# mandt-lab/PSLD

Measured on AMD Instinct MI355X. Metric: train images/sec, CIFAR-10 PSLD (6ch 32x32) NCSN++ HSM step, higher is better.
Workload: dtype f32

## Files before the change

psld_amd/csrc/conv_wino.hip:

```cpp
#include <cstdlib>
#include <cstring>
#include <type_traits>

#include "common.h"
#include "psld_hip.h"
#include "tile_shared.h"
#include "limb.h"

namespace {

constexpr int WT = 32;
constexpr int VPLANE = WT * ROWB;
constexpr int VBYTES = 16 * 3 * VPLANE;
constexpr int WINO_THREADS = 512;

struct WinoArgs {
    const float* x1;
    const float* x2;
    int C1, C2;
    int B, H, W;
    const u32x4* ufrag;
    int N, M;
    int chunks;
    float* C;
    int ldc;
    int nseg, rps;
    int cw;
    PsldEpilogue e;
    const float* zero;
    int nmajor;
    int tiles_m;
    int stagger;
    const float *gsc1, *gsh1, *gsc2, *gsh2;
    int gn_act;
    unsigned long long* dbg;
    int lg_tiles_x, lg_tps;
    int ksplit;
    long long slab_stride;
    int lg_ksplit, lg_xblocks;
    int lg_rpi;
    int mul_seg, mul_w2;
    int rb_img;
    float opscale;
};

constexpr int wino_mul16(int d) { return 65536 / d + 1; }
__host__ __device__ constexpr int wino_div16(int x, int mul) { return (x * mul) >> 16; }
constexpr int WINO_GEOS[7][2] = {{4, 4}, {4, 8}, {8, 8}, {16, 8}, {4, 16}, {8, 16}, {4, 32}};
constexpr bool wino_div16_exact() {
    for (const auto& g : WINO_GEOS) {
        const int W2 = g[1] + 2, seg_px = (g[0] + 2) * W2;
        for (int x = 0; x < 256; ++x)
            if (wino_div16(x, wino_mul16(seg_px)) != x / seg_px || wino_div16(x, wino_mul16(W2)) != x / W2) return false;
    }
    return true;
}
static_assert(wino_div16_exact(), "halo decomposition: multiply-shift must equal the division for every pixel below 256");
constexpr bool wino_geo_listed(int rps, int cw) {
    for (const auto& g : WINO_GEOS)
        if (g[0] == rps && g[1] == cw) return true;
    return false;
}
constexpr int wino_lg2(int v) {
    int l = 0;
    while ((1 << l) < v) ++l;
    return (1 << l) == v ? l : -1;
}

__device__ __forceinline__ int raw_off(int hp, int q) {
    return (hp >> 1) * 256 + (((((hp & 1) ^ ((hp >> 1) & 1)) << 3) + q) << 4);
}

template <int NL = 3>
__device__ __forceinline__ void wino_pack_item(const float* __restrict__ w, u32x4* __restrict__ out, long long it, int k_in,
                                               long long sn, long long sk, int flip) {
    const int chunks = k_in / 32;
    long long t = it;
    const int lane = (int)(t & 63); t >>= 6;
    const int chunk = (int)(t % chunks); t /= chunks;
    const int nblk = (int)t;
    const int n = nblk * 16 + (lane & 15);
    const int k0 = chunk * 32 + (lane >> 4) * 8;
    float U[8][16];
#pragma unroll
    for (int j = 0; j < 8; ++j) {
        const float* p = w + n * sn + (k0 + j) * sk;
        float g[3][3];
#pragma unroll
        for (int a = 0; a < 3; ++a)
#pragma unroll
            for (int b = 0; b < 3; ++b) g[a][b] = flip ? p[8 - (a * 3 + b)] : p[a * 3 + b];
        float t4[4][3];
#pragma unroll
        for (int b = 0; b < 3; ++b) {
            t4[0][b] = g[0][b];
            t4[1][b] = 0.5f * ((g[0][b] + g[2][b]) + g[1][b]);
            t4[2][b] = 0.5f * ((g[0][b] + g[2][b]) - g[1][b]);
            t4[3][b] = g[2][b];
        }
#pragma unroll
        for (int a = 0; a < 4; ++a) {
            U[j][a * 4 + 0] = t4[a][0];
            U[j][a * 4 + 1] = 0.5f * ((t4[a][0] + t4[a][2]) + t4[a][1]);
            U[j][a * 4 + 2] = 0.5f * ((t4[a][0] + t4[a][2]) - t4[a][1]);
            U[j][a * 4 + 3] = t4[a][2];
        }
    }
    u32x4* o = out + ((long long)nblk * chunks + chunk) * (16 * NL * 64) + lane;
#pragma unroll
    for (int p = 0; p < 16; ++p) {
        unsigned hi[4], mid[4], lo[4];
#pragma unroll
        for (int j = 0; j < 4; ++j) {
            if constexpr (NL == 3) split3(U[2 * j][p], U[2 * j + 1][p], hi[j], mid[j], lo[j]);
            else if constexpr (NL == 2) split2(U[2 * j][p], U[2 * j + 1][p], hi[j], mid[j]);
            else hi[j] = cvt_pk_f16(U[2 * j][p], U[2 * j + 1][p]);
        }
        o[(p * NL + 0) * 64] = u32x4{hi[0], hi[1], hi[2], hi[3]};
        if constexpr (NL >= 2) o[(p * NL + 1) * 64] = u32x4{mid[0], mid[1], mid[2], mid[3]};
        if constexpr (NL == 3) o[(p * 3 + 2) * 64] = u32x4{lo[0], lo[1], lo[2], lo[3]};
    }
}

template <int NL = 3>
__global__ void wino_pack_kernel(const float* __restrict__ w, u32x4* __restrict__ out, int n_out, int k_in,
                                 long long sn, long long sk, int flip) {
    const long long items = (long long)(n_out / 16) * (k_in / 32) * 64;
    for (long long it = (long long)blockIdx.x * blockDim.x + threadIdx.x; it < items; it += (long long)gridDim.x * blockDim.x)
        wino_pack_item<NL>(w, out, it, k_in, sn, sk, flip);
}

template <int NL = 3>
__global__ void wino_pack_batch_kernel(const long long* __restrict__ tab, int ntab, long long total) {
    for (long long idx = (long long)blockIdx.x * blockDim.x + threadIdx.x; idx < total;
         idx += (long long)gridDim.x * blockDim.x) {
        int lo = 0, hi = ntab - 1;
        while (lo < hi) {
            const int mid = (lo + hi + 1) >> 1;
            if (tab[8 * mid + 7] <= idx) lo = mid; else hi = mid - 1;
        }
        const long long* d = tab + 8 * lo;
        wino_pack_item<NL>(reinterpret_cast<const float*>(d[0]), reinterpret_cast<u32x4*>(d[1]), idx - d[7], (int)d[3], d[5], d[6],
                       (int)d[4]);
    }
}

template <int ABL = 0, bool GNF = false, bool ERAW = false, int LA = 2, bool TAIL = false, int NL = 3, bool SH = false>
__global__ void __launch_bounds__(WINO_THREADS) wino_conv8s_kernel(const WinoArgs a) {
    extern __shared__ __attribute__((aligned(16))) unsigned char smem[];
    constexpr int NI = 4;
    constexpr int RAWB = NI * 64 * 128;
    unsigned char* Vs = smem;
    unsigned char* Rs = smem + VBYTES / 3 * NL;

    const int tid = threadIdx.x;
    const int lane = tid & 63, wave = __builtin_amdgcn_readfirstlane(tid >> 6);
    const int tiles_n = TAIL ? (a.N + 127) >> 7 : a.N >> 7;
    const int nsp = a.ksplit > 1 ? a.ksplit : 1;
    const int tiles_m = a.tiles_m;
    const int per_range = tiles_m * tiles_n;
    const int vb = xcd_remap(blockIdx.x, gridDim.x);
    const int split = nsp > 1 ? vb / per_range : 0;
    const int bid = vb - split * per_range;
    const int kch = a.chunks >> a.lg_ksplit, ch0 = split * kch;
    float* const Cw = a.C + split * a.slab_stride;
    const int tile_n = a.nmajor ? bid / tiles_m : bid % tiles_n;
    const int tile_m = a.nmajor ? bid - tile_n * tiles_m : bid / tiles_n;
    const int n0 = tile_n * 128;
    const bool live = !TAIL || n0 + wave * 16 < a.N;

    const int HW = a.H * a.W;
    const int W2 = a.cw + 2;
    const int lg_tx = a.lg_tiles_x, lg_tps = a.lg_tps;
    const int rpi = HW >= 128 ? HW >> 7 : 1;
    const int tm_img = a.lg_rpi >= 0 ? tile_m >> a.lg_rpi : tile_m / rpi;
    const int reg = tile_m - tm_img * rpi;
    const int img0 = HW >= 128 ? tm_img : tile_m * a.nseg;
    const int oy0 = (reg >> a.lg_xblocks) * a.rps, ox0 = (reg & ((1 << a.lg_xblocks) - 1)) * a.cw;
    const float* zp = a.zero;

    const int c4 = tid & 7;
    int hoff[NI], rdst[NI];
    {
        const int seg_px = (a.rps + 2) * W2;
#pragma unroll
        for (int i = 0; i < NI; ++i) {
            const int px = (tid + WINO_THREADS * i) >> 3;
            const int seg = wino_div16(px, a.mul_seg);
            const int rem = px - seg * seg_px;
            const int hr = wino_div16(rem, a.mul_w2), hx = rem - hr * W2;
            const int img = img0 + seg, iy = oy0 + hr - 1, ix = ox0 + hx - 1;
            const bool ok = seg < a.nseg && img < a.B && iy >= 0 && iy < a.H && ix >= 0 && ix < a.W;
            hoff[i] = ok ? (img * a.H + iy) * a.W + ix : -1;
            rdst[i] = raw_off(px, c4);
        }
    }
    f32x4 hv[NI];
    auto load_raw = [&](int c) {
        const int c0 = c * 32;
        const bool second = c0 >= a.C1;
        const float* src = second ? a.x2 : a.x1;
        const int cs = second ? a.C2 : a.C1;
        const int cc = (second ? c0 - a.C1 : c0) + c4 * 4;
#pragma unroll
        for (int i = 0; i < NI; ++i) hv[i] = ld4(hoff[i] >= 0 ? src + ((long long)hoff[i] * cs + cc) : zp);
    };
    auto store_raw = [&](int buf, int c) {
        if constexpr (GNF) {
            const int c0 = c * 32;
            const bool second = c0 >= a.C1;
            const int cs = second ? a.C2 : a.C1;
            const long long go = (long long)img0 * cs + (second ? c0 - a.C1 : c0) + c4 * 4;
            const f32x4 sc = ld4((second ? a.gsc2 : a.gsc1) + go), sh = ld4((second ? a.gsh2 : a.gsh1) + go);
#pragma unroll
            for (int i = 0; i < NI; ++i) {
                f32x4 o;
#pragma unroll
                for (int e = 0; e < 4; ++e) {
                    const float z = hv[i][e] * sc[e] + sh[e];
                    const float v = a.gn_act ? silu_f(z) : z;
                    o[e] = hoff[i] >= 0 ? v : 0.f;
                }
                *reinterpret_cast<f32x4*>(Rs + buf * RAWB + rdst[i]) = o;
            }
        } else {
#pragma unroll
            for (int i = 0; i < NI; ++i) *reinterpret_cast<f32x4*>(Rs + buf * RAWB + rdst[i]) = hv[i];
        }
    };

    const int vr = wave >> 2;
    const int t_tile = (tid & 255) >> 3, t_q = tid & 7;
    int t_src;
    {
        const int seg = t_tile >> lg_tps, rem = t_tile & ((1 << lg_tps) - 1);
        const int ty = rem >> lg_tx, tx = rem & ((1 << lg_tx) - 1);
        t_src = seg < a.nseg ? (seg * (a.rps + 2) + 2 * ty) * W2 + 2 * tx : 0;
    }
    const int t_dst = t_tile * ROWB + (((t_q >> 1) ^ lds_swz(t_tile)) << 4) + (t_q & 1) * 8;
    int t_ro[3][4];
#pragma unroll
    for (int k = 0; k < 3; ++k)
#pragma unroll
        for (int c = 0; c < 4; ++c) {
            t_ro[k][c] = raw_off(t_src + (vr + k) * W2 + c, t_q);
            asm volatile("" : "+v"(t_ro[k][c]));
        }
    auto transform = [&](auto TH, auto VR, int rbuf) {
        constexpr int th = decltype(TH)::value, v_r = decltype(VR)::value;
        constexpr int ra_ = th == 0 ? (v_r == 0 ? 0 : 1) : (v_r == 0 ? 2 : 1);
        constexpr int rb_ = th == 0 ? 2 : (v_r == 0 ? 1 : 3);
        constexpr bool plus = th == 0 && v_r == 1;
        constexpr int vrow = 2 * th + v_r;
        const unsigned char* Rb = Rs + rbuf * RAWB;
        f32x4 ea[4], eb[4];
#pragma unroll
        for (int c = 0; c < 4; ++c) {
            ea[c] = *reinterpret_cast<const f32x4*>(Rb + t_ro[ra_ - v_r][c]);
            eb[c] = *reinterpret_cast<const f32x4*>(Rb + t_ro[rb_ - v_r][c]);
        }
        f32x4 r[4];
#pragma unroll
        for (int c = 0; c < 4; ++c) r[c] = plus ? ea[c] + eb[c] : ea[c] - eb[c];
#pragma unroll
        for (int j = 0; j < 4; ++j) {
            const f32x4 v = j == 0 ? r[0] - r[2] : j == 1 ? r[1] + r[2] : j == 2 ? r[2] - r[1] : r[1] - r[3];
            unsigned h0, m0_, l0, h1, m1, l1;
            if constexpr (NL == 3) {
                split3(v[0], v[1], h0, m0_, l0);
                split3(v[2], v[3], h1, m1, l1);
            } else if constexpr (NL == 2) {
                split2(v[0], v[1], h0, m0_);
                split2(v[2], v[3], h1, m1);
            } else if constexpr (SH) {
                h0 = cvt_pk_f16(v[0] * a.opscale, v[1] * a.opscale);
                h1 = cvt_pk_f16(v[2] * a.opscale, v[3] * a.opscale);
            } else {
                h0 = cvt_pk_f16(v[0], v[1]);
                h1 = cvt_pk_f16(v[2], v[3]);
            }
            unsigned char* q = Vs + (vrow * 4 + j) * NL * VPLANE + t_dst;
            *reinterpret_cast<u32x2*>(q) = u32x2{h0, h1};
            if constexpr (NL >= 2) *reinterpret_cast<u32x2*>(q + VPLANE) = u32x2{m0_, m1};
            if constexpr (NL == 3) *reinterpret_cast<u32x2*>(q + 2 * VPLANE) = u32x2{l0, l1};
        }
    };

    const int r16 = lane & 15, kq = lane >> 4;
    int aoff[2];
#pragma unroll
    for (int tb = 0; tb < 2; ++tb) {
        const int row = tb * 16 + r16;
        aoff[tb] = row * ROWB + ((kq ^ lds_swz(row)) << 4);
    }
    const u32x4* ub = a.ufrag + ((long long)(tile_n * 8 + ((ABL & 128) ? (wave & 3) : wave)) * a.chunks + ch0) * (16 * NL * 64);
    u32x4 bq[4][NL];
    auto load_b = [&](int sigma, u32x4 (&dst)[NL]) {
        const u32x4* p = ub + (long long)sigma * (NL * 64);
#pragma unroll
        for (int l = 0; l < NL; ++l) dst[l] = p[l * 64 + lane];
    };
    f32x4v acc[16][2];
#pragma unroll
    for (int p = 0; p < 16; ++p)
#pragma unroll
        for (int tb = 0; tb < 2; ++tb) acc[p][tb] = f32x4v{0.f, 0.f, 0.f, 0.f};
    u32x4 fa[NL == 1 ? 2 : NL][2];
    auto read_a = [&](int p, int l) {
#pragma unroll
        for (int tb = 0; tb < 2; ++tb) fa[l][tb] = *reinterpret_cast<const u32x4*>(Vs + (p * NL + l) * VPLANE + aoff[tb]);
    };
    auto mm = [&](int p, int la, int lb) {
#pragma unroll
        for (int tb = 0; tb < 2; ++tb) {
            if constexpr (NL == 1)
                acc[p][tb] = __builtin_amdgcn_mfma_f32_16x16x32_f16(
                    __builtin_bit_cast(f16x8, bq[p & 3][lb]), __builtin_bit_cast(f16x8, fa[la][tb]), acc[p][tb], 0, 0, 0);
            else
                acc[p][tb] = __builtin_amdgcn_mfma_f32_16x16x32_bf16(
                    __builtin_bit_cast(bf16x8, bq[p & 3][lb]), __builtin_bit_cast(bf16x8, fa[la][tb]), acc[p][tb], 0, 0, 0);
        }
    };
    auto mfma_half = [&](auto HH, auto LAST, int c) {
        constexpr int h = decltype(HH)::value;
        constexpr bool last = decltype(LAST)::value;
        if constexpr ((ABL & 256) != 0) __builtin_amdgcn_s_setprio(2);
        if constexpr (NL == 1) {
            auto read_a1 = [&](int p) {
#pragma unroll
                for (int tb = 0; tb < 2; ++tb) fa[p & 1][tb] = *reinterpret_cast<const u32x4*>(Vs + p * VPLANE + aoff[tb]);
            };
            read_a1(8 * h);
#pragma unroll
            for (int i = 0; i < 8; ++i) {
                const int p = 8 * h + i;
                if (!(last && p + LA >= 16)) load_b(c * 16 + p + LA, bq[(p + LA) & 3]);
                if (i < 7) read_a1(p + 1);
                __builtin_amdgcn_sched_barrier(0);
                mm(p, p & 1, 0);
                __builtin_amdgcn_sched_barrier(0);
            }
            return;
        }
        if constexpr (NL == 3) read_a(8 * h, 2);
        if constexpr (NL >= 2) read_a(8 * h, 1);
        read_a(8 * h, 0);
#pragma unroll
        for (int i = 0; i < 8; ++i) {
            const int p = 8 * h + i;
            if (!(ABL & 2) && !(last && p + LA >= 16)) load_b(c * 16 + p + LA, bq[(p + LA) & 3]);
            __builtin_amdgcn_sched_barrier(0);
            if constexpr (NL == 3) {
                mm(p, 2, 0);
                __builtin_amdgcn_sched_barrier(0);
                if (i < 7) read_a(p + 1, 2);
                __builtin_amdgcn_sched_barrier(0);
                mm(p, 1, 1);
            }
            if constexpr (NL >= 2) {
                mm(p, 1, 0);
                __builtin_amdgcn_sched_barrier(0);
                if (i < 7) read_a(p + 1, 1);
                __builtin_amdgcn_sched_barrier(0);
            }
            if constexpr (NL == 3) mm(p, 0, 2);
            if constexpr (NL >= 2) mm(p, 0, 1);
            mm(p, 0, 0);
            __builtin_amdgcn_sched_barrier(0);
            if (i < 7) read_a(p + 1, 0);
        }
        if constexpr ((ABL & 256) != 0) __builtin_amdgcn_s_setprio(0);
    };
    using I0 = std::integral_constant<int, 0>;
    using I1 = std::integral_constant<int, 1>;
    if constexpr ((ABL & 4) == 0 && (ABL & 256) == 0) { if (vr != 0) __builtin_amdgcn_s_setprio(1); }

    load_raw(ch0);
    if (live) {
        load_b(0, bq[0]);
        load_b(1, bq[1]);
        if (LA > 2) load_b(2, bq[2]);
    }
    store_raw(0, ch0);
    if constexpr (ERAW) load_raw(ch0 + min(1, kch - 1));
    __syncthreads();
    if (vr == 0) transform(I0{}, I0{}, 0); else transform(I0{}, I1{}, 0);
    __syncthreads();

    auto stamp = [&](int c, int idx) {
        if constexpr ((ABL & 64) != 0) {
            if (c == 3 && a.dbg) {
                __builtin_amdgcn_sched_barrier(0);
                const unsigned long long t = __builtin_amdgcn_s_memtime();
                if (lane == 0) a.dbg[((long long)blockIdx.x * 8 + wave) * 8 + idx] = t;
                __builtin_amdgcn_sched_barrier(0);
            }
        }
    };
    using No = std::false_type;
    using Yes = std::true_type;

    for (int c = 0; c < kch - 1; ++c) {
        stamp(c, 0);
        if constexpr (!ERAW) load_raw(ch0 + c + 1);
        if (vr == 0 && !(ABL & 1)) transform(I1{}, I0{}, c & 1);
        __builtin_amdgcn_sched_barrier(0);
        if (vr == 0) stamp(c, 1);
        if (live) mfma_half(I0{}, No{}, c);
        __builtin_amdgcn_sched_barrier(0);
        if (vr != 0) stamp(c, 1);
        if (vr != 0 && !(ABL & 1)) transform(I1{}, I1{}, c & 1);
        stamp(c, 2);
        store_raw((c + 1) & 1, ch0 + c + 1);
        stamp(c, 3);
        __syncthreads();
        stamp(c, 4);
        if (vr == 0 && !(ABL & 1)) transform(I0{}, I0{}, (c + 1) & 1);
        __builtin_amdgcn_sched_barrier(0);
        if (vr == 0) stamp(c, 5);
        if (live) mfma_half(I1{}, No{}, c);
        __builtin_amdgcn_sched_barrier(0);
        if (vr != 0) stamp(c, 5);
        if constexpr (ERAW) load_raw(ch0 + min(c + 2, kch - 1));
        if (vr != 0 && !(ABL & 1)) transform(I0{}, I1{}, (c + 1) & 1);
        stamp(c, 6);
        __syncthreads();
        stamp(c, 7);
    }
    {
        int c = kch - 1;
        asm volatile("" : "+s"(c));
        stamp(c, 0);
        if (vr == 0 && !(ABL & 1)) transform(I1{}, I0{}, c & 1);
        __builtin_amdgcn_sched_barrier(0);
        if (vr == 0) stamp(c, 1);
        if (live) mfma_half(I0{}, No{}, c);
        __builtin_amdgcn_sched_barrier(0);
        if (vr != 0) stamp(c, 1);
        if (vr != 0 && !(ABL & 1)) transform(I1{}, I1{}, c & 1);
        stamp(c, 2);
        stamp(c, 3);
        __syncthreads();
        stamp(c, 4);
        __builtin_amdgcn_sched_barrier(0);
        stamp(c, 5);
        if (live) mfma_half(I1{}, Yes{}, c);
        __builtin_amdgcn_sched_barrier(0);
        stamp(c, 6);
        stamp(c, 7);
    }

    if (!live) return;
    const PsldEpilogue& e = a.e;
    const int cn = n0 + wave * 16 + 4 * kq;
    const int org = (img0 * a.H + oy0) * a.W + ox0;
    const f32x4v zero4 = {0.f, 0.f, 0.f, 0.f};
    const bool rb_div = e.rowbias && !a.rb_img;
    char* const c_b = reinterpret_cast<char*>(Cw + (long long)org * a.ldc);
    const char* const res_b = reinterpret_cast<const char*>(e.res ? e.res + (long long)org * e.ldres : zp);
    f32x4v epi_bias, epi_tbv[2], epi_rv[2][4], epi_cv[2][4];
    int epi_rel[2];
    bool epi_ok[2];
    auto epi_rows = [&](auto TB) {
        constexpr int tb = decltype(TB)::value;
#pragma unroll
        for (int j = 0; j < 4; ++j) {
            const int px = epi_rel[tb] + (j >> 1) * a.W + (j & 1);
            epi_rv[tb][j] = e.res ? *reinterpret_cast<const f32x4v*>(res_b + (unsigned)((px * e.ldres + cn) * 4)) : zero4;
            epi_cv[tb][j] = e.accumulate ? *reinterpret_cast<const f32x4v*>(c_b + (unsigned)((px * a.ldc + cn) * 4)) : zero4;
        }
    };
    auto epi_request = [&]() {
        epi_bias = e.bias ? *reinterpret_cast<const f32x4v*>(e.bias + cn) : zero4;
#pragma unroll
        for (int tb = 0; tb < 2; ++tb) {
            const int tile = tb * 16 + r16;
            const int seg = tile >> lg_tps, rem = tile & ((1 << lg_tps) - 1);
            const int ty = rem >> lg_tx, tx = rem & ((1 << lg_tx) - 1);
            epi_ok[tb] = seg < a.nseg && img0 + seg < a.B;
            epi_rel[tb] = epi_ok[tb] ? seg * HW + 2 * ty * a.W + 2 * tx : 0;
            epi_tbv[tb] = a.rb_img ? *reinterpret_cast<const f32x4v*>(
                                         e.rowbias + (long long)(epi_ok[tb] ? img0 + seg : img0) * e.ld_rowbias + cn)
                                   : zero4;
        }
        epi_rows(I0{});
    };
    epi_request();
    epi_rows(I1{});
    const f32x4v bias4 = epi_bias;
#pragma unroll
    for (int tb = 0; tb < 2; ++tb) {
        const bool ok = epi_ok[tb];
        const int rel = epi_rel[tb];
#pragma unroll
        for (int i = 0; i < 4; ++i) {
            const f32x4v s0 = (acc[4 * i][tb] + acc[4 * i + 1][tb]) + acc[4 * i + 2][tb];
            acc[4 * i + 1][tb] = (acc[4 * i + 1][tb] - acc[4 * i + 2][tb]) - acc[4 * i + 3][tb];
            acc[4 * i][tb] = s0;
        }
        const f32x4v add4 = bias4 + epi_tbv[tb];
        f32x4v o[2][2];
#pragma unroll
        for (int ya = 0; ya < 2; ++ya)
#pragma unroll
            for (int xb = 0; xb < 2; ++xb) {
                const f32x4v y = ya == 0 ? (acc[xb][tb] + acc[4 + xb][tb]) + acc[8 + xb][tb]
                                         : (acc[4 + xb][tb] - acc[8 + xb][tb]) - acc[12 + xb][tb];
                f32x4v addv = add4;
                if (rb_div)
                    addv = bias4 + *reinterpret_cast<const f32x4v*>(
                                       e.rowbias + (long long)((org + rel + ya * a.W + xb) / e.rows_per_img) * e.ld_rowbias + cn);
                f32x4v x = y * e.alpha + addv;
                if (e.res) x += epi_rv[tb][ya * 2 + xb];
                x *= e.out_scale;
                if (e.accumulate) x += epi_cv[tb][ya * 2 + xb];
                o[ya][xb] = x;
            }
        const bool gn_on = e.gn_part != nullptr;
        double gs = 0.0, gss = 0.0;
        if (ok) {
#pragma unroll
            for (int ya = 0; ya < 2; ++ya)
#pragma unroll
                for (int xb = 0; xb < 2; ++xb) {
                    const int px = rel + ya * a.W + xb;
                    if ((ABL & 8) && org + px != 0) continue;
                    *reinterpret_cast<f32x4v*>(c_b + (unsigned)((px * a.ldc + cn) * 4)) = o[ya][xb];
                    if (gn_on) {
#pragma unroll
                        for (int v = 0; v < 4; ++v) {
                            const double d = (double)o[ya][xb][v];
                            gs += d;
                            gss = fma(d, d, gss);
                        }
                    }
                }
        }
        if (gn_on) {
            double s1 = gs, s2 = gss;
#pragma unroll
            for (int sft = 1; sft <= 8; sft <<= 1) {
                s1 += __shfl_xor(s1, sft, 64);
                s2 += __shfl_xor(s2, sft, 64);
            }
            const double q1 = s1, q2 = s2;
            s1 += __shfl_xor(s1, 16, 64);
            s2 += __shfl_xor(s2, 16, 64);
            const int img = a.nseg == 1 ? img0 : img0 + tb, chunk = a.nseg == 1 ? 2 * reg + tb : 0, chunks = e.gn_hw >> 6;
            if (e.gn_fine == 4) {
                if ((lane & 0xf) == 0 && img < a.B) {
                    const int f = ((n0 + wave * 16) >> 2) + (lane >> 4);
                    double* pp = e.gn_part + (((long long)img * chunks + chunk) * (a.N >> 2) + f) * 2;
                    pp[0] = q1;
                    pp[1] = q2;
                }
            } else if ((lane & 0x1f) == 0 && img < a.B) {
                const int f = ((n0 + wave * 16) >> 3) + (lane >> 5);
                double* pp = e.gn_part + (((long long)img * chunks + chunk) * (a.N >> 3) + f) * 2;
                pp[0] = s1;
                pp[1] = s2;
            }
        }
    }
}

#ifdef PSLD_ABLATIONS
#include "conv_wino_abl.inc"
#endif

inline int wino_tiles_m(int batch, int h, int w, int nseg) {
    return h * w >= 128 ? (int)cdiv((long long)batch * h * w, 128) : (int)cdiv(batch, nseg);
}

template <int ABL = 0, bool GNF = false, bool ERAW = false, int LA = 2, bool TAIL = false, int NL = 3, bool SH = false>
int launch_wino8s(const WinoArgs& a, hipStream_t stream, const char* name) {
    constexpr size_t LDS = (size_t)VBYTES / 3 * NL + 2 * (size_t)4 * 64 * 128;
    static_assert(LDS <= 163840, "LDS budget");
    if (int st = psld_lds_once<&wino_conv8s_kernel<ABL, GNF, ERAW, LA, TAIL, NL, SH>>(LDS, name)) return st;
    PSLD_CHECK_ARG(a.tiles_m == wino_tiles_m(a.B, a.H, a.W, a.nseg) && (1 << a.lg_ksplit) == (a.ksplit > 1 ? a.ksplit : 1),
                   "%s: launch geometry not filled in (tiles_m %d, ksplit %d)", name, a.tiles_m, a.ksplit);
    dim3 grid((unsigned)(a.tiles_m * cdiv(a.N, 128) * (a.ksplit > 1 ? a.ksplit : 1)));
    hipLaunchKernelGGL((wino_conv8s_kernel<ABL, GNF, ERAW, LA, TAIL, NL, SH>), grid, dim3(WINO_THREADS), LDS, stream, a);
    PSLD_CHECK_LAUNCH(name);
    return PSLD_OK;
}

int wino_cu_count() {
    static int n[PSLD_MAX_DEVICES] = {};
    int& cu = n[psld_device_slot()];
    if (cu <= 0) {
        int dev = 0;
        if (hipGetDevice(&dev) != hipSuccess || hipDeviceGetAttribute(&cu, hipDeviceAttributeMultiprocessorCount, dev) != hipSuccess ||
            cu <= 0)
            cu = 256;
    }
    return cu;
}

bool wino_geometry(int h, int w, int* nseg, int* rps, int* halo_px) {
    if (w == 128) {
        *nseg = 1; *rps = 4; *halo_px = 6 * 34;
        return h % 4 == 0;
    }
    if (w == 4) {
        *nseg = 7; *rps = 4; *halo_px = 7 * 36;
        return h == 4;
    }
    if (w != 8 && w != 16 && w != 32 && w != 64) return false;
    if (h % 2) return false;
    const int hw = h * w;
    if (hw >= 128) {
        if (hw % 128) return false;
        *nseg = 1;
        *rps = 128 / w;
    } else {
        if (128 % hw) return false;
        *nseg = 128 / hw;
        *rps = h;
    }
    if (*rps % 2) return false;
    *halo_px = *nseg * (*rps + 2) * (w + 2);
    return w == 64 ? h % 4 == 0 : *halo_px <= 256;
}

}

extern "C" long long psld_conv3x3_wino_frag_bytes(int cout, int cin) { return (long long)cout * cin * 16 * 6 + 16384; }
extern "C" long long psld_conv3x3_wino_frag_bytes_x3(int cout, int cin) { return (long long)cout * cin * 16 * 4 + 16384; }

extern "C" long long psld_conv3x3_wino_frag_bytes_f16(int cout, int cin) { return (long long)cout * cin * 16 * 2 + 16384; }

extern "C" int psld_conv3x3_wino_supported(int c1, int c2, int batch, int h, int w, int cout) {
    int nseg, rps, halo;
    return c1 > 0 && c2 >= 0 && c1 % 32 == 0 && c2 % 32 == 0 && cout >= 128 && cout % 32 == 0 && batch > 0 &&
           wino_geometry(h, w, &nseg, &rps, &halo);
}

extern "C" int psld_pack_conv3x3_wino(const float* w_oihw, void* ufrag, int cout, int cin, int dgrad, hipStream_t stream) {
    PSLD_CHECK_ARG(w_oihw && ufrag && aligned16(ufrag), "psld_pack_conv3x3_wino: null / unaligned pointer");
    const int n_out = dgrad ? cin : cout, k_in = dgrad ? cout : cin;
    PSLD_CHECK_ARG(n_out >= 128 && k_in > 0 && n_out % 32 == 0 && k_in % 32 == 0,
                   "psld_pack_conv3x3_wino: needs out channels %%32 (>= 128) and in channels %%32 (got %d, %d)", n_out, k_in);
    const long long items = (long long)(n_out / 16) * (k_in / 32) * 64;
    const unsigned blocks = psld_grid_blocks(items, 64, 16384);
    if (dgrad) hipLaunchKernelGGL(wino_pack_kernel<3>, dim3(blocks), dim3(64), 0, stream, w_oihw, reinterpret_cast<u32x4*>(ufrag),
                                  n_out, k_in, 9LL, (long long)cin * 9, 1);
    else hipLaunchKernelGGL(wino_pack_kernel<3>, dim3(blocks), dim3(64), 0, stream, w_oihw, reinterpret_cast<u32x4*>(ufrag),
                            n_out, k_in, (long long)cin * 9, 9LL, 0);
    PSLD_CHECK_LAUNCH("psld_pack_conv3x3_wino");
    return PSLD_OK;
}

extern "C" int psld_pack_conv3x3_wino_x3(const float* w_oihw, void* ufrag, int cout, int cin, hipStream_t stream) {
    PSLD_CHECK_ARG(w_oihw && ufrag && aligned16(ufrag), "psld_pack_conv3x3_wino_x3: null / unaligned pointer");
    PSLD_CHECK_ARG(cout >= 128 && cin > 0 && cout % 32 == 0 && cin % 32 == 0,
                   "psld_pack_conv3x3_wino_x3: needs out channels %%32 (>= 128) and in channels %%32 (got %d, %d)", cout, cin);
    const long long items = (long long)(cout / 16) * (cin / 32) * 64;
    const unsigned blocks = psld_grid_blocks(items, 64, 16384);
    hipLaunchKernelGGL(wino_pack_kernel<2>, dim3(blocks), dim3(64), 0, stream, w_oihw, reinterpret_cast<u32x4*>(ufrag), cout, cin,
                       (long long)cin * 9, 9LL, 0);
    PSLD_CHECK_LAUNCH("psld_pack_conv3x3_wino_x3");
    return PSLD_OK;
}

extern "C" int psld_pack_conv3x3_wino_f16(const float* w_oihw, void* ufrag, int cout, int cin, hipStream_t stream) {
    PSLD_CHECK_ARG(w_oihw && ufrag && aligned16(ufrag), "psld_pack_conv3x3_wino_f16: null / unaligned pointer");
    PSLD_CHECK_ARG(cout >= 128 && cin > 0 && cout % 32 == 0 && cin % 32 == 0,
                   "psld_pack_conv3x3_wino_f16: needs out channels %%32 (>= 128) and in channels %%32 (got %d, %d)", cout, cin);
    const long long items = (long long)(cout / 16) * (cin / 32) * 64;
    const unsigned blocks = psld_grid_blocks(items, 64, 16384);
    hipLaunchKernelGGL(wino_pack_kernel<1>, dim3(blocks), dim3(64), 0, stream, w_oihw, reinterpret_cast<u32x4*>(ufrag), cout, cin,
                       (long long)cin * 9, 9LL, 0);
    PSLD_CHECK_LAUNCH("psld_pack_conv3x3_wino_f16");
    return PSLD_OK;
}

extern "C" int psld_pack_conv3x3_wino_dgrad_f16(const float* w_oihw, void* ufrag, int cout, int cin, hipStream_t stream) {
    PSLD_CHECK_ARG(w_oihw && ufrag && aligned16(ufrag), "psld_pack_conv3x3_wino_dgrad_f16: null / unaligned pointer");
    PSLD_CHECK_ARG(cin >= 128 && cout > 0 && cin % 32 == 0 && cout % 32 == 0,
                   "psld_pack_conv3x3_wino_dgrad_f16: needs in channels %%32 (>= 128) and out channels %%32 (got %d, %d)", cin, cout);
    const long long items = (long long)(cin / 16) * (cout / 32) * 64;
    hipLaunchKernelGGL(wino_pack_kernel<1>, dim3(psld_grid_blocks(items, 64, 16384)), dim3(64), 0, stream, w_oihw,
                       reinterpret_cast<u32x4*>(ufrag), cin, cout, 9LL, (long long)cin * 9, 1);
    PSLD_CHECK_LAUNCH("psld_pack_conv3x3_wino_dgrad_f16");
    return PSLD_OK;
}

extern "C" int psld_pack_conv3x3_wino_dgrad_x3(const float* w_oihw, void* ufrag, int cout, int cin, hipStream_t stream) {
    PSLD_CHECK_ARG(w_oihw && ufrag && aligned16(ufrag), "psld_pack_conv3x3_wino_dgrad_x3: null / unaligned pointer");
    PSLD_CHECK_ARG(cin >= 128 && cout > 0 && cin % 32 == 0 && cout % 32 == 0,
                   "psld_pack_conv3x3_wino_dgrad_x3: needs in channels %%32 (>= 128) and out channels %%32 (got %d, %d)", cin, cout);
    const long long items = (long long)(cin / 16) * (cout / 32) * 64;
    hipLaunchKernelGGL(wino_pack_kernel<2>, dim3(psld_grid_blocks(items, 64, 16384)), dim3(64), 0, stream, w_oihw,
                       reinterpret_cast<u32x4*>(ufrag), cin, cout, 9LL, (long long)cin * 9, 1);
    PSLD_CHECK_LAUNCH("psld_pack_conv3x3_wino_dgrad_x3");
    return PSLD_OK;
}

extern "C" int psld_pack_wino_batch_x3(const long long* table_dev, int entries, long long total_items, hipStream_t stream) {
    PSLD_CHECK_ARG(table_dev && entries > 0 && total_items > 0, "psld_pack_wino_batch_x3: bad args");
    hipLaunchKernelGGL(wino_pack_batch_kernel<2>, dim3(psld_grid_blocks(total_items, 64, 32768)), dim3(64), 0, stream,
                       table_dev, entries, total_items);
    PSLD_CHECK_LAUNCH("psld_pack_wino_batch_x3");
    return PSLD_OK;
}

extern "C" int psld_pack_wino_batch_f16(const long long* table_dev, int entries, long long total_items, hipStream_t stream) {
    PSLD_CHECK_ARG(table_dev && entries > 0 && total_items > 0, "psld_pack_wino_batch_f16: bad args");
    hipLaunchKernelGGL(wino_pack_batch_kernel<1>, dim3(psld_grid_blocks(total_items, 64, 32768)), dim3(64), 0, stream,
                       table_dev, entries, total_items);
    PSLD_CHECK_LAUNCH("psld_pack_wino_batch_f16");
    return PSLD_OK;
}

extern "C" int psld_pack_wino_batch(const long long* table_dev, int entries, long long total_items, hipStream_t stream) {
    PSLD_CHECK_ARG(table_dev && entries > 0 && total_items > 0, "psld_pack_wino_batch: bad args");
    hipLaunchKernelGGL(wino_pack_batch_kernel<3>, dim3(psld_grid_blocks(total_items, 64, 32768)), dim3(64), 0, stream,
                       table_dev, entries, total_items);
    PSLD_CHECK_LAUNCH("psld_pack_wino_batch");
    return PSLD_OK;
}

#ifdef PSLD_ABLATIONS
static unsigned long long* g_wino_dbg = nullptr;
extern "C" void psld_abl_set_wino_debug(unsigned long long* p) { g_wino_dbg = p; }
#endif

namespace {
struct WinoGn {
    const float *sc1, *sh1, *sc2, *sh2;
    int act;
};
int wino_conv(const float* x1, int c1, const float* x2, int c2, int batch, int h, int w, const void* ufrag, int cout, float* y,
              int ldy, const psld_epilogue_t* epi, const WinoGn* gn, void* workspace, long long ws_bytes, hipStream_t stream,
              int nl = 3, int shift = -1);
}

extern "C" int psld_conv3x3_wino_f32(const float* x1, int c1, const float* x2, int c2, int batch, int h, int w,
                                     const void* ufrag, int cout, float* y, int ldy, const psld_epilogue_t* epi,
                                     hipStream_t stream) {
    return wino_conv(x1, c1, x2, c2, batch, h, w, ufrag, cout, y, ldy, epi, nullptr, nullptr, 0, stream);
}

extern "C" int psld_conv3x3_wino_ksplit(int c1, int c2, int batch, int h, int w, int cout) {
    if (!psld_conv3x3_wino_supported(c1, c2, batch, h, w, cout)) return 1;
    int nseg, rps, halo;
    wino_geometry(h, w, &nseg, &rps, &halo);
    const int tiles = wino_tiles_m(batch, h, w, nseg) * cdiv(cout, 128), chunks = (c1 + c2) / 32;
    const int cus = wino_cu_count();
    int ks = 1;
    while (tiles * ks * 2 <= cus && chunks % (ks * 2) == 0 && chunks / (ks * 2) >= 2) ks *= 2;
    return ks;
}
extern "C" long long psld_conv3x3_wino_ws_bytes(int c1, int c2, int batch, int h, int w, int cout) {
    const int ks = psld_conv3x3_wino_ksplit(c1, c2, batch, h, w, cout);
    return ks > 1 ? (long long)ks * batch * h * w * cout * 4 : 0;
}

extern "C" int psld_conv3x3_wino_ws_f32(const float* x1, int c1, const float* x2, int c2, int batch, int h, int w,
                                        const void* ufrag, int cout, float* y, int ldy, const psld_epilogue_t* epi,
                                        void* workspace, long long ws_bytes, hipStream_t stream) {
    return wino_conv(x1, c1, x2, c2, batch, h, w, ufrag, cout, y, ldy, epi, nullptr, workspace, ws_bytes, stream);
}

extern "C" int psld_conv3x3_wino_gn_supported(int c1, int c2, int batch, int h, int w, int cout) {
    return psld_conv3x3_wino_supported(c1, c2, batch, h, w, cout) && h * w >= 128 && cout % 128 == 0;
}

extern "C" int psld_conv3x3_wino_gn_f32(const float* x1, int c1, const float* scale1, const float* shift1, const float* x2,
                                        int c2, const float* scale2, const float* shift2, int act, int batch, int h, int w,
                                        const void* ufrag, int cout, float* y, int ldy, const psld_epilogue_t* epi,
                                        hipStream_t stream) {
    PSLD_CHECK_ARG(scale1 && shift1 && (c2 == 0 || (scale2 && shift2)), "psld_conv3x3_wino_gn_f32: null scale / shift");
    PSLD_CHECK_ARG(psld_conv3x3_wino_gn_supported(c1, c2, batch, h, w, cout),
                   "psld_conv3x3_wino_gn_f32: unsupported shape c1=%d c2=%d %dx%d cout=%d (needs h*w >= 128)", c1, c2, h, w, cout);
    PSLD_CHECK_ARG(aligned16(scale1) && aligned16(shift1) && (c2 == 0 || (aligned16(scale2) && aligned16(shift2))),
                   "psld_conv3x3_wino_gn_f32: unaligned scale / shift");
    const WinoGn gn{scale1, shift1, scale2, shift2, act};
    return wino_conv(x1, c1, x2, c2, batch, h, w, ufrag, cout, y, ldy, epi, &gn, nullptr, 0, stream);
}

extern "C" int psld_conv3x3_wino_gn_ws_f32(const float* x1, int c1, const float* scale1, const float* shift1, const float* x2,
                                           int c2, const float* scale2, const float* shift2, int act, int batch, int h, int w,
                                           const void* ufrag, int cout, float* y, int ldy, const psld_epilogue_t* epi,
                                           void* workspace, long long ws_bytes, hipStream_t stream) {
    PSLD_CHECK_ARG(scale1 && shift1 && (c2 == 0 || (scale2 && shift2)), "psld_conv3x3_wino_gn_ws_f32: null scale / shift");
    PSLD_CHECK_ARG(psld_conv3x3_wino_gn_supported(c1, c2, batch, h, w, cout),
                   "psld_conv3x3_wino_gn_ws_f32: unsupported shape c1=%d c2=%d %dx%d cout=%d (needs h*w >= 128)", c1, c2, h, w, cout);
    PSLD_CHECK_ARG(aligned16(scale1) && aligned16(shift1) && (c2 == 0 || (aligned16(scale2) && aligned16(shift2))),
                   "psld_conv3x3_wino_gn_ws_f32: unaligned scale / shift");
    const WinoGn gn{scale1, shift1, scale2, shift2, act};
    return wino_conv(x1, c1, x2, c2, batch, h, w, ufrag, cout, y, ldy, epi, &gn, workspace, ws_bytes, stream);
}

extern "C" int psld_conv3x3_wino_x3_f32(const float* x1, int c1, const float* x2, int c2, int batch, int h, int w,
                                        const void* ufrag, int cout, float* y, int ldy, const psld_epilogue_t* epi,
                                        void* workspace, long long ws_bytes, hipStream_t stream) {
    return wino_conv(x1, c1, x2, c2, batch, h, w, ufrag, cout, y, ldy, epi, nullptr, workspace, ws_bytes, stream, 2);
}

extern "C" int psld_conv3x3_wino_gn_x3_f32(const float* x1, int c1, const float* scale1, const float* shift1, const float* x2,
                                           int c2, const float* scale2, const float* shift2, int act, int batch, int h, int w,
                                           const void* ufrag, int cout, float* y, int ldy, const psld_epilogue_t* epi,
                                           void* workspace, long long ws_bytes, hipStream_t stream) {
    PSLD_CHECK_ARG(scale1 && shift1 && (c2 == 0 || (scale2 && shift2)), "psld_conv3x3_wino_gn_x3_f32: null scale / shift");
    PSLD_CHECK_ARG(psld_conv3x3_wino_gn_supported(c1, c2, batch, h, w, cout),
                   "psld_conv3x3_wino_gn_x3_f32: unsupported shape c1=%d c2=%d %dx%d cout=%d (needs h*w >= 128)", c1, c2, h, w, cout);
    PSLD_CHECK_ARG(aligned16(scale1) && aligned16(shift1) && (c2 == 0 || (aligned16(scale2) && aligned16(shift2))),
                   "psld_conv3x3_wino_gn_x3_f32: unaligned scale / shift");
    const WinoGn gn{scale1, shift1, scale2, shift2, act};
    return wino_conv(x1, c1, x2, c2, batch, h, w, ufrag, cout, y, ldy, epi, &gn, workspace, ws_bytes, stream, 2);
}

extern "C" int psld_conv3x3_wino_f16_f32(const float* x1, int c1, const float* x2, int c2, int batch, int h, int w,
                                         const void* ufrag, int cout, float* y, int ldy, const psld_epilogue_t* epi,
                                         void* workspace, long long ws_bytes, hipStream_t stream) {
    return wino_conv(x1, c1, x2, c2, batch, h, w, ufrag, cout, y, ldy, epi, nullptr, workspace, ws_bytes, stream, 1);
}

extern "C" int psld_conv3x3_wino_gn_f16_f32(const float* x1, int c1, const float* scale1, const float* shift1, const float* x2,
                                            int c2, const float* scale2, const float* shift2, int act, int batch, int h, int w,
                                            const void* ufrag, int cout, float* y, int ldy, const psld_epilogue_t* epi,
                                            void* workspace, long long ws_bytes, hipStream_t stream) {
    PSLD_CHECK_ARG(scale1 && shift1 && (c2 == 0 || (scale2 && shift2)), "psld_conv3x3_wino_gn_f16_f32: null scale / shift");
    PSLD_CHECK_ARG(psld_conv3x3_wino_gn_supported(c1, c2, batch, h, w, cout),
                   "psld_conv3x3_wino_gn_f16_f32: unsupported shape c1=%d c2=%d %dx%d cout=%d (needs h*w >= 128)", c1, c2, h, w, cout);
    PSLD_CHECK_ARG(aligned16(scale1) && aligned16(shift1) && (c2 == 0 || (aligned16(scale2) && aligned16(shift2))),
                   "psld_conv3x3_wino_gn_f16_f32: unaligned scale / shift");
    const WinoGn gn{scale1, shift1, scale2, shift2, act};
    return wino_conv(x1, c1, x2, c2, batch, h, w, ufrag, cout, y, ldy, epi, &gn, workspace, ws_bytes, stream, 1);
}

extern "C" int psld_conv3x3_wino_f16s_f32(const float* x1, int c1, const float* x2, int c2, int batch, int h, int w,
                                          const void* ufrag, int cout, float* y, int ldy, const psld_epilogue_t* epi, int shift,
                                          void* workspace, long long ws_bytes, hipStream_t stream) {
    PSLD_CHECK_ARG(shift >= 0 && shift <= 24, "psld_conv3x3_wino_f16s_f32: shift %d outside 0..24", shift);
    return wino_conv(x1, c1, x2, c2, batch, h, w, ufrag, cout, y, ldy, epi, nullptr, workspace, ws_bytes, stream, 1, shift);
}

namespace {
int wino_launch_f16(const WinoArgs& a, bool gn, hipStream_t stream) {
    if (gn) return launch_wino8s<0, true, false, 3, false, 1>(a, stream, "psld_conv3x3_wino_gn_f16_f32");
    if (a.N % 128) return launch_wino8s<0, false, false, 3, true, 1>(a, stream, "psld_conv3x3_wino_f16_f32");
    return launch_wino8s<0, false, false, 3, false, 1>(a, stream, "psld_conv3x3_wino_f16_f32");
}

int wino_launch_f16s(const WinoArgs& a, hipStream_t stream) {
    if (a.N % 128) return launch_wino8s<0, false, false, 3, true, 1, true>(a, stream, "psld_conv3x3_wino_f16s_f32");
    return launch_wino8s<0, false, false, 3, false, 1, true>(a, stream, "psld_conv3x3_wino_f16s_f32");
}

int wino_launch_x3(const WinoArgs& a, bool gn, hipStream_t stream) {
    if (gn) return launch_wino8s<0, true, false, 2, false, 2>(a, stream, "psld_conv3x3_wino_gn_x3_f32");
    if (a.N % 128) return launch_wino8s<0, false, false, 2, true, 2>(a, stream, "psld_conv3x3_wino_x3_f32");
    return launch_wino8s<0, false, false, 2, false, 2>(a, stream, "psld_conv3x3_wino_x3_f32");
}

int wino_conv(const float* x1, int c1, const float* x2, int c2, int batch, int h, int w, const void* ufrag, int cout, float* y,
              int ldy, const psld_epilogue_t* epi, const WinoGn* gn, void* workspace, long long ws_bytes, hipStream_t stream,
              int nl, int shift) {
    PSLD_CHECK_ARG(x1 && ufrag && y && (c2 == 0 || x2), "psld_conv3x3_wino_f32: null pointer");
    PSLD_CHECK_ARG(psld_conv3x3_wino_supported(c1, c2, batch, h, w, cout),
                   "psld_conv3x3_wino_f32: unsupported shape c1=%d c2=%d %dx%d cout=%d", c1, c2, h, w, cout);
    PSLD_CHECK_ARG(aligned16(x1) && (!x2 || aligned16(x2)) && aligned16(ufrag), "psld_conv3x3_wino_f32: unaligned pointer");
    WinoArgs a{};
    a.x1 = x1; a.x2 = x2; a.C1 = c1; a.C2 = c2;
    a.B = batch; a.H = h; a.W = w;
    a.ufrag = reinterpret_cast<const u32x4*>(ufrag);
    a.N = cout; a.M = batch * h * w;
    a.chunks = (c1 + c2) / 32;
    a.C = y; a.ldc = ldy;
    int halo_px = 0;
    wino_geometry(h, w, &a.nseg, &a.rps, &halo_px);
    a.e = make_epilogue(epi);
    if (shift >= 0) {
        a.opscale = ldexpf(1.f, shift);
        a.e.alpha *= ldexpf(1.f, -shift);
    }
    const PsldEpilogue& e = a.e;
    PSLD_CHECK_ARG(!e.gn_part || (e.gn_hw == h * w && e.gn_hw % 64 == 0 && !e.accumulate && cout % 128 == 0),
                   "psld_conv3x3_wino_f32: gn_part needs gn_hw = h*w, a multiple of 64, no accumulation and cout %% 128 == 0");
    PSLD_CHECK_ARG(ldy % 4 == 0 && aligned16(y) && (!e.res || (e.ldres % 4 == 0 && aligned16(e.res))) &&
                       (!e.bias || aligned16(e.bias)) && (!e.rowbias || (e.ld_rowbias % 4 == 0 && aligned16(e.rowbias))),
                   "limb kernels: y, residual, bias and rowbias need 16-byte aligned rows (pointer and row stride)");
    PSLD_CHECK_ARG(ldy > 0 && ldy < (1 << 20) && (!e.res || (e.ldres > 0 && e.ldres < (1 << 20))),
                   "psld_conv3x3_wino_*: row strides of y and the residual must be below 2^20 elements");
    a.zero = psld_detail_zero_page("psld_conv3x3_wino_f32");
    if (!a.zero) return PSLD_ERR_LAUNCH;
    a.nmajor = 1;
    const char* name = "psld_conv3x3_wino_f32";
    a.cw = w;
    if (w >= 64) {
        a.cw = 32; a.rps = 4; a.nseg = 1;
        halo_px = 6 * 34;
    }
    a.tiles_m = wino_tiles_m(batch, h, w, a.nseg);
    a.lg_tiles_x = wino_lg2(a.cw >> 1);
    a.lg_tps = wino_lg2((a.rps >> 1) * (a.cw >> 1));
    a.lg_xblocks = wino_lg2(w / a.cw);
    a.lg_rpi = h * w >= 128 ? wino_lg2((h * w) >> 7) : 0;
    a.lg_ksplit = 0;
    a.mul_seg = wino_mul16((a.rps + 2) * (a.cw + 2));
    a.mul_w2 = wino_mul16(a.cw + 2);
    a.rb_img = e.rowbias && e.rows_per_img == h * w;
    PSLD_CHECK_ARG(wino_geo_listed(a.rps, a.cw) && a.lg_tiles_x >= 0 && a.lg_tps >= 0 && a.lg_xblocks >= 0,
                   "psld_conv3x3_wino_*: no divisor table for the geometry of %dx%d", h, w);
    if (gn) {
        a.gsc1 = gn->sc1; a.gsh1 = gn->sh1; a.gsc2 = gn->sc2; a.gsh2 = gn->sh2; a.gn_act = gn->act;
    }
    const int ks = workspace ? psld_conv3x3_wino_ksplit(c1, c2, batch, h, w, cout) : 1;
    if (ks > 1 && (!e.gn_part || psld_detail_conv_reduce_gn_ok(a.M, cout, e)) && ws_bytes >= (long long)ks * a.M * cout * 4 && aligned16(workspace)) {
        WinoArgs s = a;
        s.ksplit = ks;
        s.lg_ksplit = wino_lg2(ks);
        s.rb_img = 0;
        s.slab_stride = (long long)a.M * cout;
        s.C = reinterpret_cast<float*>(workspace);
        s.ldc = cout;
        s.e = make_epilogue(nullptr);
        const int rc = shift >= 0 ? wino_launch_f16s(s, stream)
                       : nl == 1 ? wino_launch_f16(s, gn != nullptr, stream)
                       : nl == 2 ? wino_launch_x3(s, gn != nullptr, stream)
                       : gn    ? launch_wino8s<0, true>(s, stream, "psld_conv3x3_wino_gn_f32")
                               : (cout % 128 ? launch_wino8s<0, false, false, 2, true>(s, stream, name) : launch_wino8s<0>(s, stream, name));
        if (rc != PSLD_OK) return rc;
        return psld_detail_conv_reduce_epilogue(s.C, ks, a.M, cout, y, ldy, e, stream);
    }
    if (shift >= 0) return wino_launch_f16s(a, stream);
    if (nl == 1) return wino_launch_f16(a, gn != nullptr, stream);
    if (nl == 2) return wino_launch_x3(a, gn != nullptr, stream);
    if (gn) return launch_wino8s<0, true>(a, stream, "psld_conv3x3_wino_gn_f32");
    if (cout % 128) return launch_wino8s<0, false, false, 2, true>(a, stream, name);
#ifdef PSLD_ABLATIONS
#include "conv_wino_abl_dispatch.inc"
#endif
    return launch_wino8s<0>(a, stream, name);
}
}
```

Measured before the change: 1265.

## Stage Winograd weight packing through LDS with coalesced loads and 256-thread blocks

Rewrites the Winograd filter-transform pack kernels so each 256-thread block cooperatively loads a 16x32-channel weight tile into shared memory, using vectorized loads when aligned. The four row transforms are then split across four waves, so each thread computes a quarter of the 16 outputs. The old version issued strided scalar global loads from every thread. This targets the per-step weight repacking cost in training, in exchange for LDS use and extra barriers.

Result: no change. 1269 (median of 6 runs) (+0.3%).

```diff
diff --git a/psld_amd/csrc/conv_wino.hip b/psld_amd/csrc/conv_wino.hip
--- a/psld_amd/csrc/conv_wino.hip
+++ b/psld_amd/csrc/conv_wino.hip
@@ -71,77 +71,100 @@
     return (hp >> 1) * 256 + (((((hp & 1) ^ ((hp >> 1) & 1)) << 3) + q) << 4);
 }
 
+constexpr int PACK_THREADS = 256;
+constexpr int PACK_RS = 292, PACK_RS_FLIP = 144;
+constexpr int PACK_LDS = 16 * PACK_RS;
+
 template <int NL = 3>
-__device__ __forceinline__ void wino_pack_item(const float* __restrict__ w, u32x4* __restrict__ out, long long it, int k_in,
-                                               long long sn, long long sk, int flip) {
+__device__ __forceinline__ void wino_pack_block(const float* __restrict__ w, u32x4* __restrict__ out, long long blk, int tid,
+                                                int k_in, long long sn, long long sk, int flip, float* __restrict__ lds) {
     const int chunks = k_in / 32;
-    long long t = it;
-    const int lane = (int)(t & 63); t >>= 6;
-    const int chunk = (int)(t % chunks); t /= chunks;
-    const int nblk = (int)t;
-    const int n = nblk * 16 + (lane & 15);
-    const int k0 = chunk * 32 + (lane >> 4) * 8;
-    float U[8][16];
+    const int chunk = (int)(blk % chunks);
+    const int nblk = (int)(blk / chunks);
+    const int lane = tid & 63, a = tid >> 6;
+    const float* base = w + (long long)nblk * 16 * sn + (long long)chunk * 32 * sk;
+    const long long srow = flip ? sk : sn, scol = flip ? sn : sk;
+    const int run = flip ? 144 : 288, rs = flip ? PACK_RS_FLIP : PACK_RS;
+    if (scol == 9 && (srow & 3) == 0 && (reinterpret_cast<unsigned long long>(base) & 15) == 0) {
+        const int lgw = flip ? 5 : 6, lgr = flip ? 2 : 3;
+        const int ra = tid >> lgw, ca = tid & ((1 << lgw) - 1), rb = tid >> lgr, cb = (1 << lgw) + (tid & ((1 << lgr) - 1));
+        const float* pa = base + ra * srow + 4 * ca;
+        float* la = lds + ra * rs + 4 * ca;
+        const int na = PACK_THREADS >> lgw;
+        f32x4 v[5];
+#pragma unroll
+        for (int u = 0; u < 4; ++u) v[u] = ld4(pa + u * na * srow);
+        if (tid < 128) v[4] = ld4(base + rb * srow + 4 * cb);
+#pragma unroll
+        for (int u = 0; u < 4; ++u) *reinterpret_cast<f32x4*>(la + u * na * rs) = v[u];
+        if (tid < 128) *reinterpret_cast<f32x4*>(lds + rb * rs + 4 * cb) = v[4];
+    } else {
+#pragma unroll 6
+        for (int t = 0; t < 18; ++t) {
+            const int e = tid + PACK_THREADS * t, r = flip ? e / 144 : e / 288, c = e - r * run, x = c / 9;
+            lds[r * rs + c] = base[r * srow + x * scol + (c - 9 * x)];
+        }
+    }
+    __syncthreads();
+    const float* src = flip ? lds + (lane >> 4) * 8 * PACK_RS_FLIP + (lane & 15) * 9 + 8 : lds + (lane & 15) * PACK_RS + (lane >> 4) * 72;
+    const int sj = flip ? PACK_RS_FLIP : 9, sq = flip ? -1 : 1;
+    float g[8][9];
+#pragma unroll
+    for (int j = 0; j < 8; ++j)
+#pragma unroll
+        for (int q = 0; q < 9; ++q) g[j][q] = src[j * sj + q * sq];
+    __syncthreads();
+    float U[8][4];
 #pragma unroll
     for (int j = 0; j < 8; ++j) {
-        const float* p = w + n * sn + (k0 + j) * sk;
-        float g[3][3];
-#pragma unroll
-        for (int a = 0; a < 3; ++a)
-#pragma unroll
-            for (int b = 0; b < 3; ++b) g[a][b] = flip ? p[8 - (a * 3 + b)] : p[a * 3 + b];
-        float t4[4][3];
+        float t[3];
 #pragma unroll
         for (int b = 0; b < 3; ++b) {
-            t4[0][b] = g[0][b];
-            t4[1][b] = 0.5f * ((g[0][b] + g[2][b]) + g[1][b]);
-            t4[2][b] = 0.5f * ((g[0][b] + g[2][b]) - g[1][b]);
-            t4[3][b] = g[2][b];
-        }
-#pragma unroll
-        for (int a = 0; a < 4; ++a) {
-            U[j][a * 4 + 0] = t4[a][0];
-            U[j][a * 4 + 1] = 0.5f * ((t4[a][0] + t4[a][2]) + t4[a][1]);
-            U[j][a * 4 + 2] = 0.5f * ((t4[a][0] + t4[a][2]) - t4[a][1]);
-            U[j][a * 4 + 3] = t4[a][2];
-        }
-    }
-    u32x4* o = out + ((long long)nblk * chunks + chunk) * (16 * NL * 64) + lane;
-#pragma unroll
-    for (int p = 0; p < 16; ++p) {
+            const float s = g[j][b] + g[j][6 + b];
+            t[b] = a == 0 ? g[j][b] : a == 3 ? g[j][6 + b] : a == 1 ? 0.5f * (s + g[j][3 + b]) : 0.5f * (s - g[j][3 + b]);
+        }
+        U[j][0] = t[0];
+        U[j][1] = 0.5f * ((t[0] + t[2]) + t[1]);
+        U[j][2] = 0.5f * ((t[0] + t[2]) - t[1]);
+        U[j][3] = t[2];
+    }
+    u32x4* o = out + ((long long)nblk * chunks + chunk) * (16 * NL * 64) + a * (4 * NL * 64) + lane;
+#pragma unroll
+    for (int c = 0; c < 4; ++c) {
         unsigned hi[4], mid[4], lo[4];
 #pragma unroll
         for (int j = 0; j < 4; ++j) {
-            if constexpr (NL == 3) split3(U[2 * j][p], U[2 * j + 1][p], hi[j], mid[j], lo[j]);
-            else if constexpr (NL == 2) split2(U[2 * j][p], U[2 * j + 1][p], hi[j], mid[j]);
-            else hi[j] = cvt_pk_f16(U[2 * j][p], U[2 * j + 1][p]);
-        }
-        o[(p * NL + 0) * 64] = u32x4{hi[0], hi[1], hi[2], hi[3]};
-        if constexpr (NL >= 2) o[(p * NL + 1) * 64] = u32x4{mid[0], mid[1], mid[2], mid[3]};
-        if constexpr (NL == 3) o[(p * 3 + 2) * 64] = u32x4{lo[0], lo[1], lo[2], lo[3]};
+            if constexpr (NL == 3) split3(U[2 * j][c], U[2 * j + 1][c], hi[j], mid[j], lo[j]);
+            else if constexpr (NL == 2) split2(U[2 * j][c], U[2 * j + 1][c], hi[j], mid[j]);
+            else hi[j] = cvt_pk_f16(U[2 * j][c], U[2 * j + 1][c]);
+        }
+        o[(c * NL + 0) * 64] = u32x4{hi[0], hi[1], hi[2], hi[3]};
+        if constexpr (NL >= 2) o[(c * NL + 1) * 64] = u32x4{mid[0], mid[1], mid[2], mid[3]};
+        if constexpr (NL == 3) o[(c * 3 + 2) * 64] = u32x4{lo[0], lo[1], lo[2], lo[3]};
     }
 }
 
 template <int NL = 3>
-__global__ void wino_pack_kernel(const float* __restrict__ w, u32x4* __restrict__ out, int n_out, int k_in,
-                                 long long sn, long long sk, int flip) {
-    const long long items = (long long)(n_out / 16) * (k_in / 32) * 64;
-    for (long long it = (long long)blockIdx.x * blockDim.x + threadIdx.x; it < items; it += (long long)gridDim.x * blockDim.x)
-        wino_pack_item<NL>(w, out, it, k_in, sn, sk, flip);
+__global__ __launch_bounds__(PACK_THREADS) void wino_pack_kernel(const float* __restrict__ w, u32x4* __restrict__ out, int n_out,
+                                                                 int k_in, long long sn, long long sk, int flip) {
+    __shared__ __attribute__((aligned(16))) float lds[PACK_LDS];
+    const long long blocks = (long long)(n_out / 16) * (k_in / 32);
+    for (long long blk = blockIdx.x; blk < blocks; blk += gridDim.x)
+        wino_pack_block<NL>(w, out, blk, (int)threadIdx.x, k_in, sn, sk, flip, lds);
 }
 
 template <int NL = 3>
-__global__ void wino_pack_batch_kernel(const long long* __restrict__ tab, int ntab, long long total) {
-    for (long long idx = (long long)blockIdx.x * blockDim.x + threadIdx.x; idx < total;
-         idx += (long long)gridDim.x * blockDim.x) {
+__global__ __launch_bounds__(PACK_THREADS) void wino_pack_batch_kernel(const long long* __restrict__ tab, int ntab, long long total) {
+    __shared__ __attribute__((aligned(16))) float lds[PACK_LDS];
+    for (long long idx = (long long)blockIdx.x * 64; idx < total; idx += (long long)gridDim.x * 64) {
         int lo = 0, hi = ntab - 1;
         while (lo < hi) {
             const int mid = (lo + hi + 1) >> 1;
             if (tab[8 * mid + 7] <= idx) lo = mid; else hi = mid - 1;
         }
         const long long* d = tab + 8 * lo;
-        wino_pack_item<NL>(reinterpret_cast<const float*>(d[0]), reinterpret_cast<u32x4*>(d[1]), idx - d[7], (int)d[3], d[5], d[6],
-                       (int)d[4]);
+        wino_pack_block<NL>(reinterpret_cast<const float*>(d[0]), reinterpret_cast<u32x4*>(d[1]), (idx - d[7]) >> 6,
+                            (int)threadIdx.x, (int)d[3], d[5], d[6], (int)d[4], lds);
     }
 }
 
@@ -643,9 +666,9 @@
                    "psld_pack_conv3x3_wino: needs out channels %%32 (>= 128) and in channels %%32 (got %d, %d)", n_out, k_in);
     const long long items = (long long)(n_out / 16) * (k_in / 32) * 64;
     const unsigned blocks = psld_grid_blocks(items, 64, 16384);
-    if (dgrad) hipLaunchKernelGGL(wino_pack_kernel<3>, dim3(blocks), dim3(64), 0, stream, w_oihw, reinterpret_cast<u32x4*>(ufrag),
+    if (dgrad) hipLaunchKernelGGL(wino_pack_kernel<3>, dim3(blocks), dim3(PACK_THREADS), 0, stream, w_oihw, reinterpret_cast<u32x4*>(ufrag),
                                   n_out, k_in, 9LL, (long long)cin * 9, 1);
-    else hipLaunchKernelGGL(wino_pack_kernel<3>, dim3(blocks), dim3(64), 0, stream, w_oihw, reinterpret_cast<u32x4*>(ufrag),
+    else hipLaunchKernelGGL(wino_pack_kernel<3>, dim3(blocks), dim3(PACK_THREADS), 0, stream, w_oihw, reinterpret_cast<u32x4*>(ufrag),
                             n_out, k_in, (long long)cin * 9, 9LL, 0);
     PSLD_CHECK_LAUNCH("psld_pack_conv3x3_wino");
     return PSLD_OK;
@@ -657,7 +680,7 @@
                    "psld_pack_conv3x3_wino_x3: needs out channels %%32 (>= 128) and in channels %%32 (got %d, %d)", cout, cin);
     const long long items = (long long)(cout / 16) * (cin / 32) * 64;
     const unsigned blocks = psld_grid_blocks(items, 64, 16384);
-    hipLaunchKernelGGL(wino_pack_kernel<2>, dim3(blocks), dim3(64), 0, stream, w_oihw, reinterpret_cast<u32x4*>(ufrag), cout, cin,
+    hipLaunchKernelGGL(wino_pack_kernel<2>, dim3(blocks), dim3(PACK_THREADS), 0, stream, w_oihw, reinterpret_cast<u32x4*>(ufrag), cout, cin,
                        (long long)cin * 9, 9LL, 0);
     PSLD_CHECK_LAUNCH("psld_pack_conv3x3_wino_x3");
     return PSLD_OK;
@@ -669,7 +692,7 @@
                    "psld_pack_conv3x3_wino_f16: needs out channels %%32 (>= 128) and in channels %%32 (got %d, %d)", cout, cin);
     const long long items = (long long)(cout / 16) * (cin / 32) * 64;
     const unsigned blocks = psld_grid_blocks(items, 64, 16384);
-    hipLaunchKernelGGL(wino_pack_kernel<1>, dim3(blocks), dim3(64), 0, stream, w_oihw, reinterpret_cast<u32x4*>(ufrag), cout, cin,
+    hipLaunchKernelGGL(wino_pack_kernel<1>, dim3(blocks), dim3(PACK_THREADS), 0, stream, w_oihw, reinterpret_cast<u32x4*>(ufrag), cout, cin,
                        (long long)cin * 9, 9LL, 0);
     PSLD_CHECK_LAUNCH("psld_pack_conv3x3_wino_f16");
     return PSLD_OK;
@@ -680,7 +703,7 @@
     PSLD_CHECK_ARG(cin >= 128 && cout > 0 && cin % 32 == 0 && cout % 32 == 0,
                    "psld_pack_conv3x3_wino_dgrad_f16: needs in channels %%32 (>= 128) and out channels %%32 (got %d, %d)", cin, cout);
     const long long items = (long long)(cin / 16) * (cout / 32) * 64;
-    hipLaunchKernelGGL(wino_pack_kernel<1>, dim3(psld_grid_blocks(items, 64, 16384)), dim3(64), 0, stream, w_oihw,
+    hipLaunchKernelGGL(wino_pack_kernel<1>, dim3(psld_grid_blocks(items, 64, 16384)), dim3(PACK_THREADS), 0, stream, w_oihw,
                        reinterpret_cast<u32x4*>(ufrag), cin, cout, 9LL, (long long)cin * 9, 1);
     PSLD_CHECK_LAUNCH("psld_pack_conv3x3_wino_dgrad_f16");
     return PSLD_OK;
@@ -691,7 +714,7 @@
     PSLD_CHECK_ARG(cin >= 128 && cout > 0 && cin % 32 == 0 && cout % 32 == 0,
                    "psld_pack_conv3x3_wino_dgrad_x3: needs in channels %%32 (>= 128) and out channels %%32 (got %d, %d)", cin, cout);
     const long long items = (long long)(cin / 16) * (cout / 32) * 64;
-    hipLaunchKernelGGL(wino_pack_kernel<2>, dim3(psld_grid_blocks(items, 64, 16384)), dim3(64), 0, stream, w_oihw,
+    hipLaunchKernelGGL(wino_pack_kernel<2>, dim3(psld_grid_blocks(items, 64, 16384)), dim3(PACK_THREADS), 0, stream, w_oihw,
                        reinterpret_cast<u32x4*>(ufrag), cin, cout, 9LL, (long long)cin * 9, 1);
     PSLD_CHECK_LAUNCH("psld_pack_conv3x3_wino_dgrad_x3");
     return PSLD_OK;
@@ -699,7 +722,7 @@
 
 extern "C" int psld_pack_wino_batch_x3(const long long* table_dev, int entries, long long total_items, hipStream_t stream) {
     PSLD_CHECK_ARG(table_dev && entries > 0 && total_items > 0, "psld_pack_wino_batch_x3: bad args");
-    hipLaunchKernelGGL(wino_pack_batch_kernel<2>, dim3(psld_grid_blocks(total_items, 64, 32768)), dim3(64), 0, stream,
+    hipLaunchKernelGGL(wino_pack_batch_kernel<2>, dim3(psld_grid_blocks(total_items, 64, 32768)), dim3(PACK_THREADS), 0, stream,
                        table_dev, entries, total_items);
     PSLD_CHECK_LAUNCH("psld_pack_wino_batch_x3");
     return PSLD_OK;
@@ -707,7 +730,7 @@
 
 extern "C" int psld_pack_wino_batch_f16(const long long* table_dev, int entries, long long total_items, hipStream_t stream) {
     PSLD_CHECK_ARG(table_dev && entries > 0 && total_items > 0, "psld_pack_wino_batch_f16: bad args");
-    hipLaunchKernelGGL(wino_pack_batch_kernel<1>, dim3(psld_grid_blocks(total_items, 64, 32768)), dim3(64), 0, stream,
+    hipLaunchKernelGGL(wino_pack_batch_kernel<1>, dim3(psld_grid_blocks(total_items, 64, 32768)), dim3(PACK_THREADS), 0, stream,
                        table_dev, entries, total_items);
     PSLD_CHECK_LAUNCH("psld_pack_wino_batch_f16");
     return PSLD_OK;
@@ -715,7 +738,7 @@
 
 extern "C" int psld_pack_wino_batch(const long long* table_dev, int entries, long long total_items, hipStream_t stream) {
     PSLD_CHECK_ARG(table_dev && entries > 0 && total_items > 0, "psld_pack_wino_batch: bad args");
-    hipLaunchKernelGGL(wino_pack_batch_kernel<3>, dim3(psld_grid_blocks(total_items, 64, 32768)), dim3(64), 0, stream,
+    hipLaunchKernelGGL(wino_pack_batch_kernel<3>, dim3(psld_grid_blocks(total_items, 64, 32768)), dim3(PACK_THREADS), 0, stream,
                        table_dev, entries, total_items);
     PSLD_CHECK_LAUNCH("psld_pack_wino_batch");
     return PSLD_OK;
```
